# chacorp/latent-nerf-test

Hardware: AMD Instinct MI355X
Metric: latent-frames/sec (64x64x4, 128^3 grid), render forward+backward (higher is better)
Workload: dtype bf16

## Files before the change

include/lnerf_hip.h:

```cpp
#ifndef LNERF_HIP_H
#define LNERF_HIP_H

#include <stddef.h>
#include <stdint.h>

#ifdef __cplusplus
extern "C" {
#endif

#define LNERF_ABI_VERSION 7

#define LNERF_OK 0
#define LNERF_ERR_INVALID_ARG (-1)
#define LNERF_ERR_HIP (-2)
#define LNERF_ERR_UNSUPPORTED (-3)

#define LNERF_F32 0
#define LNERF_BF16 1

#define LNERF_MAX_LEVELS 32

typedef void *lnerf_stream_t;

int lnerf_abi_version(void);
// ... 115 lines not shown
                       float blob_scale, float blob_std, int64_t m_host, const int32_t *m_dev, const float *sigmas,
                       const float *dsigmas, const float *drgbs, float *dfeat, float *dw1, float *db1, float *dw2,
                       float *db2, float *dw3, float *db3, int accumulate, void *workspace, size_t workspace_bytes,
                       int precision, void *clear_ptr, size_t clear_bytes, lnerf_stream_t stream);

int lnerf_density_normals(const float *dxyz_enc, const float *xyzs, const float *sigmas, float blob_scale,
                          float blob_std, int64_t m_host, const int32_t *m_dev, float *grad_sigma, float *normals,
                          lnerf_stream_t stream);

int lnerf_opacity_entropy_grad(const float *weights_sum, int64_t N, float scale, float eps, float *grad,
                               lnerf_stream_t stream);

int lnerf_synthetic_guidance(const float *image, const float *targets, const int32_t *dirs, const float *weights,
                             int64_t n_views, int rays_per_view, int C, int n_buckets, int t_lo, int t_hi,
                             float noise_scale, uint32_t seed, const int32_t *step_dev, float *grad_image,
                             const float *weights_sum, float ent_scale, float ent_eps, float *grad_weights_sum,
                             lnerf_stream_t stream);

int lnerf_composite_rays_train_forward(const float *sigmas, const float *rgbs, const float *deltas,
                                       const int32_t *rays, int64_t N, int C, float T_thresh, const float *bg_color,
                                       float *weights_sum, float *depth, float *image, lnerf_stream_t stream);
int lnerf_composite_rays_train_backward(const float *grad_weights_sum, const float *grad_depth,
                                        const float *grad_image, const float *sigmas, const float *rgbs,
                                        const float *deltas, const int32_t *rays, const float *weights_sum,
                                        const float *depth, const float *image, const float *bg_color, int64_t N,
                                        int C, float T_thresh, float *grad_sigmas, float *grad_rgbs, float *grad_bg,
                                        lnerf_stream_t stream);

int lnerf_composite_rays_train_decode_forward(const float *sigmas, const float *latents, const float *deltas,
                                              const int32_t *rays, int64_t N, float T_thresh, const float *decoder,
                                              const float *bg_color, float *weights_sum, float *depth,
                                              float *latent_image, float *image, lnerf_stream_t stream);
int lnerf_composite_rays_train_decode_backward(const float *grad_weights_sum, const float *grad_depth,
                                               const float *grad_image, const float *sigmas, const float *latents,
                                               const float *deltas, const int32_t *rays, const float *weights_sum,
                                               const float *depth, const float *latent_image, const float *decoder,
                                               const float *bg_color, int64_t N, float T_thresh, float *grad_sigmas,
                                               float *grad_latents, float *grad_bg, float *grad_decoder,
                                               lnerf_stream_t stream);
int lnerf_decode_image(const float *latent_image, const float *weights_sum, const float *decoder, const float *bg_color,
                       int64_t N, float *image, lnerf_stream_t stream);

int lnerf_occ_cell_points(const uint32_t *indices, int64_t n, int cascade_level, int grid_size, float bound,
                          const float *noise, float *xyzs, lnerf_stream_t stream);
size_t lnerf_occ_sample_scratch_bytes(int64_t n_cells);
int lnerf_occ_sample(const float *grid_level, int64_t n_cells, int cascade_level, int grid_size, float bound,
                     int64_t n_rand, uint32_t seed, uint32_t step, int32_t *scratch, uint32_t *indices, float *xyzs,
                     lnerf_stream_t stream);
int lnerf_occ_update(float *grid_level, const uint32_t *indices, int64_t n, const float *new_sigmas, float decay,
                     uint32_t *scratch_cells, lnerf_stream_t stream);
int lnerf_occ_update_mean(float *grid_level, int64_t n_cells, const uint32_t *indices, int64_t n, const float *new_sigmas,
                          float decay, uint32_t *scratch_cells, float *mean_dev, float *scratch256,
                          lnerf_stream_t stream);
int lnerf_occ_mean(const float *grid, int64_t n, float *mean_dev, float *scratch256, lnerf_stream_t stream);

int lnerf_bg_forward(const float *dirs, int64_t N, const float *w1, const float *b1, const float *w2, const float *b2,
                     int C, float *out, lnerf_stream_t stream);
int lnerf_bg_backward(const float *dirs, int64_t N, const float *w1, const float *b1, const float *w2, const float *b2,
                      int C, const float *dout, float *dw1, float *db1, float *dw2, float *db2, lnerf_stream_t stream);

int lnerf_mesh_winding_number(const float *points, int64_t n, const float *triangles, int n_faces, float *out,
                              lnerf_stream_t stream);
int lnerf_mesh_distance(const float *points, int64_t n, const float *triangles, int n_faces, float *out,
                        lnerf_stream_t stream);

int lnerf_raster_prepare(const float *verts, int n_verts, const int32_t *faces, int n_faces, const float *cam_host,
                         float *face_z, float *face_xy, lnerf_stream_t stream);
int lnerf_rasterize(int H, int W, const float *face_z, const float *face_xy, int n_faces, int32_t *face_idx,
                    float *bary, lnerf_stream_t stream);
int lnerf_raster_prepare_batch(const float *verts, int n_verts, const int32_t *faces, int n_faces,
                               const float *cams_dev, int B, int H, int W, float *face_z, float *face_xy,
                               int16_t *face_box, lnerf_stream_t stream);
int lnerf_rasterize_batch(int B, int H, int W, const float *face_z, const float *face_xy, const int16_t *face_box,
                          int n_faces, int32_t *face_idx, float *bary, lnerf_stream_t stream);
int lnerf_interpolate_attributes(const int32_t *face_idx, const float *bary, const float *attr, int n_pixels, int D,
                                 float *feat, lnerf_stream_t stream);
int lnerf_interpolate_attributes_backward(const int32_t *face_idx, const float *bary, const float *dfeat,
                                          int n_pixels, int D, float *dattr, lnerf_stream_t stream);
int lnerf_texture_map_forward(const float *uv, const int32_t *face_idx, const float *texture, int n_pixels, int C,
                              int R, int mode, float *out, lnerf_stream_t stream);
int lnerf_texture_map_backward(const float *uv, const int32_t *face_idx, const float *dout, int n_pixels, int C, int R,
                               int mode, float *dtexture, lnerf_stream_t stream);

int lnerf_uv_footprint(const int32_t *face_idx, const float *face_xy, const float *face_z, const float *face_uv, int B,
                       int H, int W, int n_faces, float *rho, lnerf_stream_t stream);
int lnerf_mip_build(const float *texture, int C, int R, int L, float *pyramid, lnerf_stream_t stream);
int lnerf_mip_build_backward(float *dpyramid, int C, int R, int L, float *dtexture, lnerf_stream_t stream);
int lnerf_texture_mip_forward(const float *uv, const float *rho, const int32_t *face_idx, const float *texture,
                              const float *pyramid, int n_pixels, int C, int R, int L, float bias, float *out,
                              lnerf_stream_t stream);
int lnerf_texture_mip_backward(const float *uv, const float *rho, const int32_t *face_idx, const float *dout,
                               int n_pixels, int C, int R, int L, float bias, float *dtexture, float *dpyramid,
                               lnerf_stream_t stream);

int lnerf_adam_step(float *p, void *g, int grad_dtype, float *m, float *v, void *shadow_bf16, int64_t n, float lr,
                    float beta1, float beta2, float eps, int step, const int32_t *step_dev, float grad_scale,
                    int zero_grad, lnerf_stream_t stream);
int lnerf_adam_tick(int32_t *step_dev, lnerf_stream_t stream);
#define LNERF_ADAM_TICK 2
int lnerf_adam_step_multi(int count, float *const *p_host, float *const *g_host, float *const *m_host,
                          float *const *v_host, const int64_t *n_host, const float *lr_host, float beta1, float beta2,
                          float eps, int step, const int32_t *step_dev, float grad_scale, int zero_grad,
                          lnerf_stream_t stream);
int lnerf_adam_step_multi_shadow(int count, float *const *p_host, float *const *g_host, float *const *m_host,
                                 float *const *v_host, const int64_t *n_host, const float *lr_host, float beta1,
                                 float beta2, float eps, int step, const int32_t *step_dev, float grad_scale,
// ... 142 lines not shown
```

latent-nerf-test_amd/csrc/rays.hip:

```cpp
#include "common.h"

#include <math.h>
#include <string.h>

namespace lnerf {

__device__ __forceinline__ void pixel_ray(const float *__restrict__ c2w, int H, int W, float fx, float fy, float cx,
                                          float cy, int64_t g, float o[3], float d[3]) {
    const int b = (int)(g / ((int64_t)H * W));
    const int p = (int)(g - (int64_t)b * H * W);
    const int j = p / W, i = p - j * W;
    const float *m = c2w + (int64_t)b * 16;
    const float xs = ((float)i + 0.5f - cx) / fx;
    const float ys = ((float)j + 0.5f - cy) / fy;
    const float inv = 1.0f / sqrtf(xs * xs + ys * ys + 1.0f);
    const float d0 = xs * inv, d1 = ys * inv, d2 = inv;
#pragma unroll
    for (int r = 0; r < 3; ++r) {
        d[r] = d0 * m[r * 4 + 0] + d1 * m[r * 4 + 1] + d2 * m[r * 4 + 2];
        o[r] = m[r * 4 + 3];
    }
}
__global__ void __launch_bounds__(256) k_get_rays(const float *__restrict__ c2w, int B, int H, int W, float fx,
                                                  float fy, float cx, float cy, float *__restrict__ rays_o,
// ... 646 lines not shown
__global__ void __launch_bounds__(256) k_occ_update_apply(float *__restrict__ grid, unsigned int *__restrict__ scratch,
                                                          const uint32_t *__restrict__ indices, int64_t n, float decay) {
    for (int64_t i = (int64_t)blockIdx.x * blockDim.x + threadIdx.x; i < n; i += (int64_t)gridDim.x * blockDim.x) {
        const uint32_t idx = indices ? indices[i] : (uint32_t)i;
        const unsigned int m = atomicExch(&scratch[idx], 0u);
        if (!(m & 0x80000000u)) continue;
        const float old = grid[idx];
        if (old >= 0.f) grid[idx] = fmaxf(old * decay, __uint_as_float(m & 0x7FFFFFFFu));
    }
}

constexpr int OCC_MEAN_BLOCKS = 256;
__global__ void __launch_bounds__(256) k_occ_mean_partial(const float *__restrict__ grid, int64_t n,
                                                          float *__restrict__ partial) {
    __shared__ float s_w[4];
    float s = 0.f;
    for (int64_t i = (int64_t)blockIdx.x * blockDim.x + threadIdx.x; i < n; i += (int64_t)gridDim.x * blockDim.x)
        s += fmaxf(grid[i], 0.f);
    s = wave_sum(s);
    if (lane_id() == 0) s_w[threadIdx.x >> 6] = s;
    __syncthreads();
    if (threadIdx.x == 0) partial[blockIdx.x] = ((s_w[0] + s_w[1]) + s_w[2]) + s_w[3];
}
__global__ void __launch_bounds__(256) k_occ_apply_mean(float *__restrict__ grid, unsigned int *__restrict__ scratch,
                                                        int64_t n, float decay, float *__restrict__ partial) {
    __shared__ float s_w[4];
    float s = 0.f;
    for (int64_t i = (int64_t)blockIdx.x * blockDim.x + threadIdx.x; i < n; i += (int64_t)gridDim.x * blockDim.x) {
        float g = grid[i];
        const unsigned int m = scratch[i];
        if (m & 0x80000000u) {
            scratch[i] = 0u;
            if (g >= 0.f) {
                g = fmaxf(g * decay, __uint_as_float(m & 0x7FFFFFFFu));
                grid[i] = g;
            }
        }
        s += fmaxf(g, 0.f);
    }
    s = wave_sum(s);
    if (lane_id() == 0) s_w[threadIdx.x >> 6] = s;
    __syncthreads();
    if (threadIdx.x == 0) partial[blockIdx.x] = ((s_w[0] + s_w[1]) + s_w[2]) + s_w[3];
}
__global__ void __launch_bounds__(64) k_occ_mean_final(const float *__restrict__ partial, int blocks, float n,
                                                       float *__restrict__ mean) {
    if (threadIdx.x == 0) {
        float s = 0.f;
        for (int b = 0; b < blocks; ++b) s += partial[b];
        *mean = s / n;
    }
}

static MarchParams make_params(float bound, int cascade, int G, int max_steps, float dt_gamma) {
    MarchParams P;
    P.bound = bound;
    P.cascade = cascade;
    P.G = G;
    P.max_steps = max_steps;
    P.dt_gamma = dt_gamma;
    P.dt_min = (float)(2.0 * 1.7320508075688772 / (double)max_steps);
    P.dt_max = (float)(2.0 * 1.7320508075688772 * (double)(1 << (cascade - 1)) / (double)G);
    P.dt_uniform = fminf(fmaxf(0.0f, P.dt_min), P.dt_max);
    return P;
}

static int grid_for(int64_t n, int block = 256, int cap = 4096) {
    int64_t g = div_up(n, block);
    if (g < 1) g = 1;
    if (g > cap) g = cap;
    return (int)g;
}

}

using namespace lnerf;

extern "C" {

int lnerf_get_rays(const float *c2w, int B, int H, int W, float fx, float fy, float cx, float cy, float *rays_o,
                   float *rays_d, lnerf_stream_t stream) {
    LNERF_REQUIRE(c2w && rays_o && rays_d, "get_rays: null pointer");
    LNERF_REQUIRE(B > 0 && H > 0 && W > 0, "get_rays: B,H,W must be positive (got %d,%d,%d)", B, H, W);
    LNERF_REQUIRE(fx != 0.f && fy != 0.f, "get_rays: zero focal length");
    const int64_t total = (int64_t)B * H * W;
    hipLaunchKernelGGL(k_get_rays, dim3(grid_for(total)), dim3(256), 0, as_stream(stream), c2w, B, H, W, fx, fy, cx, cy,
                       rays_o, rays_d);
    LNERF_CHECK_LAUNCH("get_rays");
    return LNERF_OK;
}

int lnerf_near_far_from_aabb(const float *rays_o, const float *rays_d, int64_t N, float xmin, float ymin, float zmin,
                             float xmax, float ymax, float zmax, float min_near, float *nears, float *fars,
                             lnerf_stream_t stream) {
    LNERF_REQUIRE(N >= 0, "near_far_from_aabb: negative N");
    if (N == 0) return LNERF_OK;
    LNERF_REQUIRE(rays_o && rays_d && nears && fars, "near_far_from_aabb: null pointer");
    LNERF_REQUIRE(xmin <= xmax && ymin <= ymax && zmin <= zmax, "near_far_from_aabb: inverted aabb");
    const RayBox box{xmin, ymin, zmin, xmax, ymax, zmax, min_near};
    hipLaunchKernelGGL(k_near_far, dim3(grid_for(N)), dim3(256), 0, as_stream(stream), rays_o, rays_d, N, box, nears, fars);
    LNERF_CHECK_LAUNCH("near_far_from_aabb");
    return LNERF_OK;
}

int lnerf_morton3d(const int32_t *coords, int64_t n, uint32_t *indices, lnerf_stream_t stream) {
    LNERF_REQUIRE(n >= 0, "morton3d: negative n");
// ... 209 lines not shown
    if (n_rand == 0) return LNERF_OK;
    LNERF_REQUIRE(grid_level && scratch && indices && xyzs, "occ_sample: null pointer");
    const int n_blocks = (int)div_up(n_cells, (int64_t)OCC_BLOCK_CELLS);
    int32_t *counts = scratch, *total = scratch + n_blocks, *list = scratch + n_blocks + 1;
    hipStream_t s = as_stream(stream);
    hipLaunchKernelGGL(k_occ_count, dim3((unsigned)n_blocks), dim3(256), 0, s, grid_level, n_cells, counts);
    LNERF_CHECK_LAUNCH("occ_sample(count)");
    hipLaunchKernelGGL(k_occ_fill, dim3((unsigned)n_blocks), dim3(256), 0, s, grid_level, n_cells, counts, n_blocks, list, total);
    LNERF_CHECK_LAUNCH("occ_sample(fill)");
    const float mip_bound = fminf((float)(1 << cascade_level), bound);
    hipLaunchKernelGGL(k_occ_draw, dim3(grid_for(2 * n_rand)), dim3(256), 0, s, list, total, n_cells, n_rand, seed, step,
                       mip_bound, grid_size, indices, xyzs);
    LNERF_CHECK_LAUNCH("occ_sample(draw)");
    return LNERF_OK;
}

size_t lnerf_occ_sample_scratch_bytes(int64_t n_cells) {
    if (n_cells <= 0) return 0;
    return (size_t)(div_up(n_cells, (int64_t)OCC_BLOCK_CELLS) + 1 + n_cells) * sizeof(int32_t);
}

int lnerf_occ_update(float *grid_level, const uint32_t *indices, int64_t n, const float *new_sigmas, float decay,
                     uint32_t *scratch_cells, lnerf_stream_t stream) {
    LNERF_REQUIRE(n >= 0, "occ_update: negative n");
    if (n == 0) return LNERF_OK;
    LNERF_REQUIRE(grid_level && new_sigmas && scratch_cells, "occ_update: null pointer");
    hipStream_t s = as_stream(stream);
    hipLaunchKernelGGL(k_occ_update_max, dim3(grid_for(n)), dim3(256), 0, s, scratch_cells, indices, n, new_sigmas);
    LNERF_CHECK_LAUNCH("occ_update(max)");
    hipLaunchKernelGGL(k_occ_update_apply, dim3(grid_for(n)), dim3(256), 0, s, grid_level, scratch_cells, indices, n, decay);
    LNERF_CHECK_LAUNCH("occ_update(apply)");
    return LNERF_OK;
}

int lnerf_occ_update_mean(float *grid_level, int64_t n_cells, const uint32_t *indices, int64_t n, const float *new_sigmas,
                          float decay, uint32_t *scratch_cells, float *mean_dev, float *scratch256,
                          lnerf_stream_t stream) {
    LNERF_REQUIRE(n >= 0 && n_cells > 0, "occ_update_mean: bad sizes");
    LNERF_REQUIRE(grid_level && scratch_cells && mean_dev && scratch256 && (n == 0 || new_sigmas),
                  "occ_update_mean: null pointer");
    hipStream_t s = as_stream(stream);
    if (n > 0) {
        hipLaunchKernelGGL(k_occ_update_max, dim3(grid_for(n)), dim3(256), 0, s, scratch_cells, indices, n, new_sigmas);
        LNERF_CHECK_LAUNCH("occ_update_mean(max)");
    }
    hipLaunchKernelGGL(k_occ_apply_mean, dim3(OCC_MEAN_BLOCKS), dim3(256), 0, s, grid_level, scratch_cells, n_cells, decay,
                       scratch256);
    LNERF_CHECK_LAUNCH("occ_update_mean(apply)");
    hipLaunchKernelGGL(k_occ_mean_final, dim3(1), dim3(64), 0, s, scratch256, OCC_MEAN_BLOCKS, (float)n_cells, mean_dev);
    LNERF_CHECK_LAUNCH("occ_update_mean(final)");
    return LNERF_OK;
}

int lnerf_occ_mean(const float *grid, int64_t n, float *mean_dev, float *scratch256, lnerf_stream_t stream) {
    LNERF_REQUIRE(n > 0 && grid && mean_dev && scratch256, "occ_mean: bad arguments");
    hipLaunchKernelGGL(k_occ_mean_partial, dim3(OCC_MEAN_BLOCKS), dim3(256), 0, as_stream(stream), grid, n, scratch256);
    LNERF_CHECK_LAUNCH("occ_mean(partial)");
    hipLaunchKernelGGL(k_occ_mean_final, dim3(1), dim3(64), 0, as_stream(stream), scratch256, OCC_MEAN_BLOCKS, (float)n,
                       mean_dev);
    LNERF_CHECK_LAUNCH("occ_mean(final)");
    return LNERF_OK;
}

}
```

latent-nerf-test_amd/src/latent_nerf/configs/render_config.py:

```python
from typing import Optional
from dataclasses import dataclass
from typing import Tuple

from ..models.nerf_utils import NeRFType


@dataclass
class RenderConfig:
    cuda_ray: bool = True
    max_steps: int = 1024
    num_steps: int = 128
    upsample_steps: int = 0
    update_extra_interval: int = 16
    occ_device_sampling: bool = True
    max_ray_batch: int = 4096
    density_thresh: float = 10.0
    train_w: int = 64
    train_h: int = 64
    eval_w: int = 128
    eval_h: int = 128
    jitter_pose: bool = False
    bound: float = 1.0
    dt_gamma: float = 0.0
    min_near: float = 0.1
    radius_range: Tuple[float, float] = (1.0, 1.5)
    fovy_range: Tuple[float, float] = (40.0, 70.0)
    train_pose: Optional[Tuple[float, float, float, float]] = None
    dir_text: bool = True
    angle_overhead: float = 30.0
    angle_front: float = 60.0
    backbone: str = "grid"
    nerf_type: NeRFType = NeRFType.latent
    bg_radius: float = 0.0
    grid_size: int = 128
    mlp_precision: str = "auto"
    table_dtype: str = "auto"
    gridtype: str = "auto"
    gather_variant: int = 0
    scatter_variant: int = -1
    noise_seed: Optional[int] = 0x5EED
    max_samples: int = 0

    def layout(self) -> str:
        if self.gridtype not in ("auto", "hash", "tiled", "blocked"):
            raise ValueError("render.gridtype must be 'auto', 'hash', 'tiled' or 'blocked' (got %r)" % (self.gridtype,))
        return "hash" if self.gridtype == "auto" else self.gridtype

    def precision(self, name: str) -> str:
        v = getattr(self, name)
        if v not in ("auto", "f32", "bf16"):
            raise ValueError("render.%s must be 'auto', 'f32' or 'bf16' (got %r)" % (name, v))
        return "f32" if v == "auto" else v
```

latent-nerf-test_amd/src/latent_nerf/models/renderer.py:

```python
import math
import os

import torch
import torch.nn as nn

from ..raymarching import backend as _b
from ..raymarching import raymarching as rm
from ..raymarching.raymarching import _p, _stream


def _sample_pdf(bins, weights, n_samples, stratified):
    w = weights + 1e-5
    cdf = torch.cumsum(w / w.sum(-1, keepdim=True), -1)
    cdf = torch.cat([torch.zeros_like(cdf[:, :1]), cdf], -1)
    if stratified:
        u = torch.linspace(0.5 / n_samples, 1.0 - 0.5 / n_samples, n_samples, device=bins.device)
        u = u[None].expand(bins.shape[0], n_samples).contiguous()
    else:
        u = torch.rand(bins.shape[0], n_samples, device=bins.device)
    hi = torch.searchsorted(cdf, u, right=True).clamp(max=cdf.shape[-1] - 1)
    lo = (hi - 1).clamp(min=0)
    c0, c1 = torch.gather(cdf, 1, lo), torch.gather(cdf, 1, hi)
    b0, b1 = torch.gather(bins, 1, lo), torch.gather(bins, 1, hi)
    span = c1 - c0
# ... 15 lines not shown
        self.r = renderer

    def __enter__(self):
        r = self.r
        if r._shadow_state is None or r._shadow_state[0].device != r.density_grid.device:
            r._shadow_state = [getattr(r, n).clone() for n in self.NAMES]
        self.real = [r._buffers[n] for n in self.NAMES]
        for n, t in zip(self.NAMES, r._shadow_state):
            r._buffers[n] = t
        return r

    def __exit__(self, *exc):
        for n, t in zip(self.NAMES, self.real):
            self.r._buffers[n] = t
        return False


class NeRFRenderer(nn.Module):
    def __init__(self, cfg, latent_mode: bool = True):
        super().__init__()
        self.cfg = cfg
        self.latent_mode = latent_mode
        self.tuned = False
        self.bound = float(cfg.bound)
        self.cascade = 1 + math.ceil(math.log2(cfg.bound)) if cfg.bound > 1 else 1
        self.grid_size = int(cfg.grid_size)
        self.density_scale = 1.0
        self.min_near = cfg.min_near
        self.density_thresh = cfg.density_thresh
        self.bg_radius = cfg.bg_radius
        self.cuda_ray = cfg.cuda_ray
        aabb = torch.tensor([-self.bound] * 3 + [self.bound] * 3, dtype=torch.float32)
        self.register_buffer("aabb_train", aabb)
        self.register_buffer("aabb_infer", aabb.clone())
        G3 = self.grid_size ** 3
        self.register_buffer("density_grid", torch.zeros(self.cascade, G3))
        self.register_buffer("density_bitfield", torch.zeros(self.cascade * G3 // 8, dtype=torch.uint8))
        self.register_buffer("mean_density_dev", torch.zeros(1))
        self.mean_density = 0.0
        self.iter_density = 0
        self.local_step = 0
        self._march = None
        self._march_slots = [None, None]
        self._ray_slots = [None, None]
        self._march_key = None
        self._budget = None
        self.mean_count = 0
        self._noise_counter = None
        self._occ_scratch = None
        self._occ_cells = None
        self._occ_gen = None
        self._occ_seed = 0x0CC0
        self._occ_sample_ws = None
        self._bg_const = {}
        self._shadow_state = None

    def forward(self, x, d=None):
        raise NotImplementedError()

    def density(self, x):
        raise NotImplementedError()

    def field(self, xyzs, m_host, m_dev=None, level_stride=None):
        raise NotImplementedError()

    def background(self, d):
        raise NotImplementedError()

    def normal(self, x):
        raise NotImplementedError()

    def decode_points(self, latents):
        raise NotImplementedError()

    def density_normals(self, xyzs):
        raise NotImplementedError()

    SHADED = ("lambertian", "textureless")

    def _check_shading(self, shading, light_d=None, sampler="run_cuda", orient=False, normal_image=False):
        if normal_image and (shading not in self.SHADED or not self.training or sampler != "run_cuda" or self.tuned):
            raise ValueError("normal_image=True needs shading='lambertian' / 'textureless' in training mode on the "
                             "occupancy-marched renderer, not latent_tune (got shading=%r, %s mode, %s%s)"
                             % (shading, "training" if self.training else "evaluation", sampler,
                                ", latent_tune" if self.tuned else ""))
        if orient and (shading not in self.SHADED or not self.training or sampler != "run_cuda"):
            raise ValueError("orient=True needs shading='lambertian' / 'textureless' in training mode on the "
                             "occupancy-marched renderer (got shading=%r, %s mode, %s)"
                             % (shading, "training" if self.training else "evaluation", sampler))
        if shading in self.SHADED:
            if light_d is None:
                raise ValueError("shading must be 'albedo' or 'normal' unless light_d is given: shading=%r needs "
                                 "light_d=[3] / [B,3] (direction toward the light)" % (shading,))
            if sampler != "run_cuda":
                raise ValueError("shading=%r is built for the occupancy-marched renderer (cuda_ray = true); the uniform "
                                 "sampler renders 'albedo' and 'normal'" % (shading,))
            if self.tuned:
                raise ValueError("shading=%r is not available with render.nerf_type = latent_tune (the decoded colours "
                                 "are composited per ray)" % (shading,))
            return False, True
        if shading not in ("albedo", "normal"):
            raise ValueError("shading must be 'albedo', 'normal', or 'lambertian' / 'textureless' with light_d "
                             "(got %r)" % (shading,))
        if shading == "normal" and self.training:
            raise ValueError("shading='normal' is an evaluation render: call .eval() first (normals are not "
                             "differentiable here)")
# ... 425 lines not shown
        extra = {}
        if atlas == "charts":
            vt, ft, info = rm.chart_atlas(verts, faces, R)
            extra = {"face_chart": info["face_chart"], "chart_rect": info["chart_rect"], "atlas_scale": info["scale"]}
        else:
            need = atlas_min_resolution(F)
            if F > 0 and R < need:
                warnings.warn("export_mesh: texture_resolution %d gives the per-triangle atlas of %d faces %.1f texels per "
                              "chart cell (fewer than %d): use texture_resolution >= %d, or target_faces <= %d"
                              % (R, F, R / atlas_cells(F), MIN_TEXELS_PER_CELL, need, 2 * (R // MIN_TEXELS_PER_CELL) ** 2),
                              stacklevel=3)
            vt, ft = per_triangle_atlas(F, verts.device)
        baked = self.bake_texture(verts, faces, vt, ft, resolution=R, gutter=gutter, S=S)
        os.makedirs(path, exist_ok=True)
        out = os.path.join(path, "mesh.obj")
        write_textured_obj(out, verts.cpu().numpy(), faces.cpu().numpy(), vt.cpu().numpy(), ft.cpu().numpy(),
                           normals.cpu().numpy(), material="mesh.mtl", texture="albedo.png")
        albedo = (baked["rgb"].permute(1, 2, 0).cpu().numpy() * 255).round().astype(np.uint8)
        Image.fromarray(albedo).save(os.path.join(path, "albedo.png"))
        if (self.latent_mode or self.tuned) and baked["texture"].shape[0] == 4:
            torch.save(baked["texture"].cpu(), os.path.join(path, "latent_texture.pt"))
        if normal_map:
            nmap = self.bake_texture(verts, faces, vt, ft, resolution=R, gutter=gutter, S=S,
                                     fn=lambda pts: (self.normal(pts) + 1.0) / 2.0)["texture"]
            img = (nmap.clamp(0, 1).permute(1, 2, 0).cpu().numpy() * 255).round().astype(np.uint8)
            Image.fromarray(img).save(os.path.join(path, "normal_object.png"))
            baked = dict(baked, normal_map=nmap)
        return dict(baked, vt=vt, ft=ft, **extra)

    def shadow_extra_state(self):
        return _ShadowExtraState(self)

    def occupancy_generator(self, seed=None):
        dev = self.density_grid.device
        if seed is not None or self._occ_gen is None or self._occ_gen.device != dev:
            self._occ_gen = torch.Generator(device=dev)
            self._occ_gen.manual_seed(0x0CC0 + (0 if seed is None else int(seed)))
            if seed is not None:
                self._occ_seed = 0x0CC0 + int(seed)
        return self._occ_gen

    @torch.no_grad()
    def update_extra_state(self, decay=0.95, S=128):
        if not self.cuda_ray:
            return
        if self.training:
            self.update_sample_budget()
        dev = self.density_grid.device
        gen = self.occupancy_generator()
        G, G3 = self.grid_size, self.grid_size ** 3
        chunk = 1 << 20
        if self._occ_cells is None or self._occ_cells.device != dev:
            self._occ_cells = torch.zeros(G3, device=dev, dtype=torch.int32)
        fused_mean = False
        for cas in range(self.cascade):
            if self.iter_density >= 16 and getattr(self.cfg, "occ_device_sampling", True):
                n_rand = G3 // 4
                if self._occ_sample_ws is None or self._occ_sample_ws[0].device != dev:
                    nb = _b.get_lib().lnerf_occ_sample_scratch_bytes(G3)
                    self._occ_sample_ws = (torch.empty(nb, device=dev, dtype=torch.uint8),
                                           torch.empty(2 * n_rand, device=dev, dtype=torch.int32),
                                           torch.empty(2 * n_rand, 3, device=dev))
                scratch, idx, xyzs = self._occ_sample_ws
                level = self.density_grid[cas]
                _b.call("lnerf_occ_sample", _p(level), G3, cas, G, self.bound, n_rand, self._occ_seed & 0xFFFFFFFF,
                        (self.iter_density * 8 + cas) & 0xFFFFFFFF, _p(scratch), _p(idx), _p(xyzs), _stream())
                sigmas, _ = self.field(xyzs, 2 * n_rand)
                sigmas = sigmas.contiguous() if self.density_scale == 1.0 else (sigmas * self.density_scale).contiguous()
                if self.cascade == 1:
                    if self._occ_scratch is None or self._occ_scratch.device != dev:
                        self._occ_scratch = torch.zeros(256, device=dev)
                    _b.call("lnerf_occ_update_mean", _p(level), G3, _p(idx), 2 * n_rand, _p(sigmas), float(decay),
                            _p(self._occ_cells), _p(self.mean_density_dev), _p(self._occ_scratch), _stream())
                    fused_mean = True
                    continue
                _b.call("lnerf_occ_update", _p(level), _p(idx), 2 * n_rand, _p(sigmas), float(decay), _p(self._occ_cells),
                        _stream())
                continue
            if self.iter_density < 16:
                indices = None
                n = G3
            else:
                n_rand = G3 // 4
                rand_idx = torch.randint(0, G3, (n_rand,), device=dev, dtype=torch.int32, generator=gen)
                occ = torch.nonzero(self.density_grid[cas] > 0).squeeze(-1)
                if occ.numel() > 0:
                    pick = torch.randint(0, occ.numel(), (n_rand,), device=dev, generator=gen)
                    occ_idx = occ[pick].to(torch.int32)
                    indices = torch.cat([rand_idx, occ_idx])
                else:
                    indices = rand_idx
                n = indices.numel()
            level = self.density_grid[cas]
            for s in range(0, n, chunk):
                e = min(s + chunk, n)
                idx = None if indices is None else indices[s:e].contiguous()
                if idx is None:
                    idx = torch.arange(s, e, device=dev, dtype=torch.int32)
                noise = torch.rand(e - s, 3, device=dev, generator=gen)
                xyzs = torch.empty(e - s, 3, device=dev)
                _b.call("lnerf_occ_cell_points", _p(idx), e - s, cas, G, self.bound, _p(noise), _p(xyzs), _stream())
                sigmas, _ = self.field(xyzs, e - s)
                sigmas = (sigmas * self.density_scale).contiguous()
                _b.call("lnerf_occ_update", _p(level), _p(idx), e - s, _p(sigmas), float(decay), _p(self._occ_cells),
                        _stream())
        if not fused_mean:
            if self._occ_scratch is None or self._occ_scratch.device != dev:
                self._occ_scratch = torch.zeros(256, device=dev)
            _b.call("lnerf_occ_mean", _p(self.density_grid), self.density_grid.numel(), _p(self.mean_density_dev),
                    _p(self._occ_scratch), _stream())
        self.iter_density += 1
        rm.packbits(self.density_grid, self.density_thresh, self.density_bitfield, self.mean_density_dev)

    def render(self, rays_o, rays_d, staged=False, max_ray_batch=4096, **kwargs):
        _run = self.run_cuda if self.cuda_ray else self.run
        if not self.cuda_ray:
            kwargs.setdefault("num_steps", self.cfg.num_steps)
            kwargs.setdefault("upsample_steps", self.cfg.upsample_steps)
        if kwargs.get("prepared") is not None or (kwargs.get("camera") is not None and self.cuda_ray and self.training):
            kwargs.pop("force_all_rays", None)
            return self.run_cuda(None, None, **kwargs)
        camera = kwargs.pop("camera", None)
        if camera is not None and rays_o is None:
            poses, intr, him, wim = camera
            if torch.is_tensor(intr):
                intr = [float(v) for v in intr.reshape(-1)[:4].tolist()]
            rays_o, rays_d = rm.get_rays(poses, intr, int(him), int(wim))
        B, N = rays_o.shape[:2]
        if staged and not self.cuda_ray:
            dev = rays_o.device
            depth = torch.empty(B, N, device=dev)
            image = torch.empty(B, N, 3 if kwargs.get("shading", "albedo") == "normal" else self.img_dims, device=dev)
            wsum = torch.empty(B, N, device=dev)
            for b in range(B):
                for head in range(0, N, max_ray_batch):
                    tail = min(head + max_ray_batch, N)
                    r = _run(rays_o[b:b + 1, head:tail], rays_d[b:b + 1, head:tail], **kwargs)
                    depth[b:b + 1, head:tail] = r["depth"]
                    image[b:b + 1, head:tail] = r["image"]
                    wsum[b:b + 1, head:tail] = r["weights_sum"]
            return {"depth": depth, "image": image, "weights_sum": wsum}
        return _run(rays_o, rays_d, **kwargs)
```

latent-nerf-test_amd/src/latent_nerf/raymarching/backend.py:

```python
import ctypes
import os
import re

_HERE = os.path.dirname(os.path.abspath(__file__))
PKG_ROOT = os.path.abspath(os.path.join(_HERE, "..", "..", ".."))
REPO_ROOT = os.path.abspath(os.path.join(PKG_ROOT, ".."))
LIB_PATH = os.environ.get("LNERF_HIP_LIB", os.path.join(PKG_ROOT, "lib", "liblnerf_hip.so"))
HEADER_PATH = os.path.join(REPO_ROOT, "include", "lnerf_hip.h")

LNERF_OK = 0
F32, BF16 = 0, 1
MLP_FRAGMENTS_READY = 0x100
SCATTER_ZERO_HEAD_BYTES = 64 * 1024
MLP_FRAGMENT_BYTES = 36 * 1024
SCATTER_DEFER_FINISH = 0x200
MLP_DEFER_REDUCE = 0x200
TAIL_TICK, TAIL_CLEAR_SCATTER = 1, 2
GRID_BLOCKED = 0x400
GRID_TILED = 0x800
SCATTER_CLEARED = 0x100
MC_CLOSE_BOUNDARY, MC_COUNT_ONLY, MC_REUSE_COUNT = 1, 2, 4
UV_ITEMS, UV_COVER, UV_EMIT = 1, 2, 4
UV_MAX_RES = 8192
DECIMATE_DEFAULT_ROUNDS = 128
# ... 29 lines not shown
    "lnerf_build_info": [],
    "lnerf_set_tuning": [_c.c_char_p, _I],
    "lnerf_get_rays": [_P, _I, _I, _I, _F, _F, _F, _F, _P, _P, _P],
    "lnerf_near_far_from_aabb": [_P, _P, _L, _F, _F, _F, _F, _F, _F, _F, _P, _P, _P],
    "lnerf_morton3d": [_P, _L, _P, _P],
    "lnerf_morton3d_invert": [_P, _L, _P, _P],
    "lnerf_packbits": [_P, _L, _F, _P, _P, _P],
    "lnerf_march_rays_train": [_P, _P, _P, _P, _L, _P, _F, _I, _I, _I, _F, _P, _U, _P, _L, _P, _P, _P, _P, _P, _P],
    "lnerf_march_rays_train_aabb": [_P, _P, _F, _F, _F, _F, _F, _F, _F, _L, _P, _F, _I, _I, _I, _F, _P, _U, _P, _L, _P, _P,
                                    _P, _P, _P, _P],
    "lnerf_march_rays_train_pose": [_P, _I, _I, _I, _F, _F, _F, _F, _P, _P, _F, _F, _F, _F, _F, _F, _F, _P, _F, _I, _I, _I,
                                    _F, _P, _U, _P, _L, _P, _P, _P, _P, _P, _P],
    "lnerf_march_rays_train_camera": [_P, _P, _I, _I, _I, _P, _P, _F, _F, _F, _F, _F, _F, _F, _P, _F, _I, _I, _I, _F, _P, _U,
                                      _P, _L, _P, _P, _P, _P, _P, _P],
    "lnerf_march_rays": [_L, _I, _P, _P, _P, _P, _P, _P, _F, _I, _I, _I, _F, _P, _P, _P, _P],
    "lnerf_composite_rays": [_L, _I, _P, _P, _P, _P, _P, _I, _F, _P, _P, _P, _P, _P],
    "lnerf_compact_rays": [_P, _L, _P, _P, _P],
    "lnerf_grid_encode_forward": [_P, _F, _P, _I, _I, _I, _P, _P, _P, _L, _P, _L, _P, _I, _I, _P],
    "lnerf_grid_encode_backward_workspace_bytes": [_I, _P, _L],
    "lnerf_grid_encode_backward": [_P, _F, _P, _I, _I, _I, _P, _P, _P, _L, _P, _L, _P, _I, _P, _Z, _P],
    "lnerf_grid_encode_backward_bf16": [_P, _F, _P, _I, _I, _I, _P, _P, _P, _L, _P, _L, _P, _I, _P, _Z, _P, _P],
    "lnerf_grid_scatter_bin": [_P, _F, _P, _I, _I, _I, _P, _P, _P, _L, _P, _L, _P, _I, _P, _Z, _P],
    "lnerf_grid_scatter_reduce_bf16": [_F, _I, _I, _P, _P, _P, _L, _L, _I, _I, _P, _I, _P, _Z, _P, _P],
    "lnerf_grid_encode_backward_adam": [_P, _F, _P, _I, _I, _I, _P, _P, _P, _L, _P, _L, _P, _I, _P, _Z, _P, _P, _P, _P, _F,
                                        _F, _F, _F, _I, _P, _F, _P],
    "lnerf_grid_encode_backward_input": [_P, _F, _P, _I, _I, _I, _P, _P, _P, _L, _P, _L, _P, _P, _I, _P],
    "lnerf_grid_tv_plan": [_I, _P, _L, _P],
    "lnerf_grid_tv_lines": [_I, _P, _P, _U, _U, _P, _P, _P],
    "lnerf_grid_tv_grad": [_P, _I, _I, _P, _P, _I, _P, _P, _U, _U, _P, _P, _P, _P],
    "lnerf_density_normals": [_P, _P, _P, _F, _F, _L, _P, _P, _P, _P],
    "lnerf_mlp_forward": [_P, _I, _L, _P, _P, _P, _P, _P, _P, _P, _I, _F, _F, _L, _P, _P, _P, _I, _P, _Z, _P],
    "lnerf_mlp_backward_workspace_bytes": [_I],
    "lnerf_grid_scatter_clear_bytes": [_I, _P, _L],
    "lnerf_moment_map_bytes": [_I, _P],
    "lnerf_moment_map_build": [_P, _P, _I, _I, _P, _P, _Z, _P],
    "lnerf_moment_map_bind": [_P, _P, _Z],
    "lnerf_occ_sample_scratch_bytes": [_L],
    "lnerf_march_counter_len": [_L],
    "lnerf_occ_sample": [_P, _L, _I, _I, _F, _L, _U, _U, _P, _P, _P, _P],
    "lnerf_mlp_backward": [_P, _I, _L, _P, _P, _P, _P, _P, _P, _P, _I, _F, _F, _L, _P, _P, _P, _P, _P, _P, _P, _P,
                           _P, _P, _P, _I, _P, _Z, _I, _P, _Z, _P],
    "lnerf_composite_rays_train_forward": [_P, _P, _P, _P, _L, _I, _F, _P, _P, _P, _P, _P],
    "lnerf_composite_rays_train_backward": [_P, _P, _P, _P, _P, _P, _P, _P, _P, _P, _P, _L, _I, _F, _P, _P, _P, _P],
    "lnerf_composite_rays_train_decode_forward": [_P, _P, _P, _P, _L, _F, _P, _P, _P, _P, _P, _P, _P],
    "lnerf_composite_rays_train_decode_backward": [_P, _P, _P, _P, _P, _P, _P, _P, _P, _P, _P, _P, _L, _F, _P, _P, _P, _P,
                                                   _P],
    "lnerf_decode_image": [_P, _P, _P, _P, _L, _P, _P],
    "lnerf_opacity_entropy_grad": [_P, _L, _F, _F, _P, _P],
    "lnerf_synthetic_guidance": [_P, _P, _P, _P, _L, _I, _I, _I, _I, _I, _F, _U, _P, _P, _P, _F, _F, _P, _P],
    "lnerf_occ_cell_points": [_P, _L, _I, _I, _F, _P, _P, _P],
    "lnerf_occ_update": [_P, _P, _L, _P, _F, _P, _P],
    "lnerf_occ_mean": [_P, _L, _P, _P, _P],
    "lnerf_occ_update_mean": [_P, _L, _P, _L, _P, _F, _P, _P, _P, _P],
    "lnerf_bg_forward": [_P, _L, _P, _P, _P, _P, _I, _P, _P],
    "lnerf_bg_backward": [_P, _L, _P, _P, _P, _P, _I, _P, _P, _P, _P, _P, _P],
    "lnerf_mesh_winding_number": [_P, _L, _P, _I, _P, _P],
    "lnerf_mesh_distance": [_P, _L, _P, _I, _P, _P],
    "lnerf_raster_prepare": [_P, _I, _P, _I, _P, _P, _P, _P],
    "lnerf_rasterize": [_I, _I, _P, _P, _I, _P, _P, _P],
    "lnerf_raster_prepare_batch": [_P, _I, _P, _I, _P, _I, _I, _I, _P, _P, _P, _P],
    "lnerf_rasterize_batch": [_I, _I, _I, _P, _P, _P, _I, _P, _P, _P],
    "lnerf_interpolate_attributes": [_P, _P, _P, _I, _I, _P, _P],
    "lnerf_interpolate_attributes_backward": [_P, _P, _P, _I, _I, _P, _P],
    "lnerf_texture_map_forward": [_P, _P, _P, _I, _I, _I, _I, _P, _P],
    "lnerf_texture_map_backward": [_P, _P, _P, _I, _I, _I, _I, _P, _P],
    "lnerf_uv_footprint": [_P, _P, _P, _P, _I, _I, _I, _I, _P, _P],
    "lnerf_mip_build": [_P, _I, _I, _I, _P, _P],
    "lnerf_mip_build_backward": [_P, _I, _I, _I, _P, _P],
    "lnerf_texture_mip_forward": [_P, _P, _P, _P, _P, _I, _I, _I, _I, _F, _P, _P],
    "lnerf_texture_mip_backward": [_P, _P, _P, _P, _I, _I, _I, _I, _F, _P, _P, _P],
    "lnerf_adam_step": [_P, _P, _I, _P, _P, _P, _L, _F, _F, _F, _F, _I, _P, _F, _I, _P],
    "lnerf_adam_tick": [_P, _P],
    "lnerf_adam_step_multi": [_I, _P, _P, _P, _P, _P, _P, _F, _F, _F, _I, _P, _F, _I, _P],
    "lnerf_adam_step_multi_shadow": [_I, _P, _P, _P, _P, _P, _P, _F, _F, _F, _I, _P, _F, _I, _P, _P, _P],
    "lnerf_mlp_fragment_maps": [_I, _P, _P, _P, _P],
    "lnerf_cast_f32_to_bf16": [_P, _P, _L, _P],
    "lnerf_mlp_backward_slabs": [_L, _I],
    "lnerf_grid_encode_backward_adam_tail": [_P, _F, _P, _I, _I, _I, _P, _P, _P, _L, _P, _L, _P, _I, _P, _Z, _P, _P, _P, _P,
                                             _F, _P, _Z, _I, _I, _P, _P, _P, _F, _P, _F, _F, _F, _I, _P, _F, _I, _P],
    "lnerf_marching_cubes_scratch_bytes": [_I, _I, _I, _I],
    "lnerf_marching_cubes": [_P, _I, _I, _I, _F, _F, _F, _F, _F, _F, _F, _I, _P, _Z, _P, _P, _L, _P, _L, _P, _P],
    "lnerf_uv_raster_scratch_bytes": [_I, _I],
    "lnerf_uv_raster": [_P, _I, _P, _P, _I, _P, _I, _I, _I, _L, _P, _Z, _P, _P, _P, _L, _P, _P],
    "lnerf_uv_dilate": [_P, _P, _I, _I, _I, _P, _P, _P],
    "lnerf_decimate_scratch_bytes": [_I, _I],
    "lnerf_decimate": [_P, _I, _P, _I, _I, _F, _I, _P, _Z, _P, _P, _P, _P, _P],
    "lnerf_atlas_buckets": [_P, _I, _P, _I, _P, _P, _P, _P],
    "lnerf_atlas_round": [_P, _P, _I, _P, _P, _P],
    "lnerf_atlas_compact_scratch_bytes": [_I],
    "lnerf_atlas_compact": [_P, _P, _I, _P, _Z, _P, _P, _P, _P],
    "lnerf_atlas_boxes_scratch_bytes": [_I],
    "lnerf_atlas_boxes": [_P, _I, _P, _P, _P, _I, _I, _P, _Z, _P, _P],
    "lnerf_atlas_uv": [_P, _I, _P, _P, _I, _P, _P, _P, _P, _I, _I, _F, _I, _P, _I, _P],
    "lnerf_atlas_fold_scratch_bytes": [_I, _I],
    "lnerf_atlas_fold": [_P, _I, _P, _I, _I, _I, _L, _P, _Z, _P, _P, _P, _P],
    "lnerf_mesh_components_begin": [_P, _I, _I, _P, _P, _P],
    "lnerf_mesh_components_round": [_P, _I, _I, _P, _P, _P],
    "lnerf_mesh_components_scratch_bytes": [_I, _I],
    "lnerf_mesh_components_finish": [_P, _I, _P, _I, _P, _P, _Z, _P, _P, _P, _P, _P, _P],
    "lnerf_mesh_filter_scratch_bytes": [_I, _I],
    "lnerf_mesh_filter": [_P, _I, _I, _P, _P, _Z, _P, _P, _P, _P],
    "lnerf_mesh_smooth_scratch_bytes": [_I, _I],
    "lnerf_mesh_smooth": [_P, _I, _P, _I, _I, _F, _F, _P, _Z, _P, _P, _P],
    "lnerf_fd_points": [_P, _F, _F, _L, _P, _P, _P, _P],
    "lnerf_shade_fd_forward": [_P, _P, _I, _P, _L, _I, _P, _I, _F, _P, _P, _P],
    "lnerf_shade_fd_backward": [_P, _P, _I, _P, _L, _I, _P, _I, _F, _P, _P, _P, _P, _P],
# ... 87 lines not shown
```

Before: 2794.

## Use stratified pull-based occupancy update and fuse mean into packbits

```diff
diff --git a/include/lnerf_hip.h b/include/lnerf_hip.h
--- a/include/lnerf_hip.h
+++ b/include/lnerf_hip.h
@@ -191,6 +191,11 @@
 int lnerf_occ_update_mean(float *grid_level, int64_t n_cells, const uint32_t *indices, int64_t n, const float *new_sigmas,
                           float decay, uint32_t *scratch_cells, float *mean_dev, float *scratch256,
                           lnerf_stream_t stream);
+int lnerf_occ_update_mean_stratified(float *grid_level, int64_t n_cells, const uint32_t *indices, int64_t n,
+                                     const float *new_sigmas, float decay, uint32_t *scratch_cells, float *mean_dev,
+                                     float *scratch256, int64_t n_rand, const int32_t *total_dev, lnerf_stream_t stream);
+int lnerf_packbits_partials(const float *grid, int64_t n_cells, float thresh, const float *partial256, float *mean_dev,
+                            uint8_t *bitfield, lnerf_stream_t stream);
 int lnerf_occ_mean(const float *grid, int64_t n, float *mean_dev, float *scratch256, lnerf_stream_t stream);
 
 int lnerf_bg_forward(const float *dirs, int64_t N, const float *w1, const float *b1, const float *w2, const float *b2,
diff --git a/latent-nerf-test_amd/csrc/rays.hip b/latent-nerf-test_amd/csrc/rays.hip
--- a/latent-nerf-test_amd/csrc/rays.hip
+++ b/latent-nerf-test_amd/csrc/rays.hip
@@ -722,6 +722,122 @@
     }
 }
 
+__global__ void __launch_bounds__(256) k_occ_run_max(unsigned int *__restrict__ scratch,
+                                                     const uint32_t *__restrict__ indices, int64_t n_rand,
+                                                     const float *__restrict__ sig, const int32_t *__restrict__ total_dev) {
+    if (*total_dev <= 0) return;
+    const int lane = lane_id();
+    const int64_t n_up = (n_rand + 255) / 256 * 256;
+    for (int64_t k = (int64_t)blockIdx.x * blockDim.x + threadIdx.x; k < n_up; k += (int64_t)gridDim.x * blockDim.x) {
+        const bool in = k < n_rand;
+        const uint32_t idx = in ? indices[n_rand + k] : 0xFFFFFFFFu;
+        const uint32_t next = (k + 1 < n_rand) ? indices[n_rand + k + 1] : 0xFFFFFFFFu;
+        const float s = in ? sig[n_rand + k] : -1.0f;
+        unsigned int v = (s >= 0.f) ? (__float_as_uint(s) | 0x80000000u) : 0u;
+#pragma unroll
+        for (int d = 1; d < 64; d <<= 1) {
+            const unsigned int ov = (unsigned int)__shfl_up((int)v, d, 64);
+            const uint32_t oi = (uint32_t)__shfl_up((int)idx, d, 64);
+            if (lane >= d && oi == idx) v = v > ov ? v : ov;
+        }
+        if (in && v != 0u && (lane == 63 || next != idx)) atomicMax(&scratch[idx], v);
+    }
+}
+__device__ __forceinline__ unsigned int occ_pull_word(const uint32_t *__restrict__ indices, const float *__restrict__ sig,
+                                                      int64_t j, uint32_t cell) {
+    const float c = sig[j];
+    return (indices[j] == cell && c >= 0.f) ? (__float_as_uint(c) | 0x80000000u) : 0u;
+}
+__device__ __forceinline__ float occ_apply_cell(float *__restrict__ grid, unsigned int *__restrict__ scratch, int64_t i,
+                                                float g, unsigned int held, unsigned int m, float decay) {
+    m = m > held ? m : held;
+    if (held & 0x80000000u) scratch[i] = 0u;
+    if ((m & 0x80000000u) && g >= 0.f) {
+        g = fmaxf(g * decay, __uint_as_float(m & 0x7FFFFFFFu));
+        grid[i] = g;
+    }
+    return fmaxf(g, 0.f);
+}
+constexpr int OCC_APPLY_TRIPS = 8;
+template <bool SECOND>
+__device__ __forceinline__ float occ_apply_slice(float *__restrict__ grid, unsigned int *__restrict__ scratch, int64_t n,
+                                                 float decay, const uint32_t *__restrict__ indices, int64_t n_rand,
+                                                 const float *__restrict__ sig) {
+    const int64_t stride = (int64_t)gridDim.x * blockDim.x;
+    float s = 0.f;
+    int64_t i = (int64_t)blockIdx.x * blockDim.x + threadIdx.x;
+    for (; i + (OCC_APPLY_TRIPS - 1) * stride < n; i += OCC_APPLY_TRIPS * stride) {
+        float g[OCC_APPLY_TRIPS];
+        unsigned int held[OCC_APPLY_TRIPS], m[OCC_APPLY_TRIPS];
+#pragma unroll
+        for (int u = 0; u < OCC_APPLY_TRIPS; ++u) {
+            const int64_t c = i + u * stride;
+            g[u] = grid[c];
+            held[u] = scratch[c];
+            m[u] = occ_pull_word(indices, sig, c >> 2, (uint32_t)c);
+            if (SECOND) {
+                const unsigned int v = occ_pull_word(indices, sig, n_rand + (c >> 2), (uint32_t)c);
+                m[u] = m[u] > v ? m[u] : v;
+            }
+        }
+#pragma unroll
+        for (int u = 0; u < OCC_APPLY_TRIPS; ++u) s += occ_apply_cell(grid, scratch, i + u * stride, g[u], held[u], m[u], decay);
+    }
+    for (; i < n; i += stride) {
+        unsigned int m = occ_pull_word(indices, sig, i >> 2, (uint32_t)i);
+        if (SECOND) {
+            const unsigned int v = occ_pull_word(indices, sig, n_rand + (i >> 2), (uint32_t)i);
+            m = m > v ? m : v;
+        }
+        s += occ_apply_cell(grid, scratch, i, grid[i], scratch[i], m, decay);
+    }
+    return s;
+}
+__global__ void __launch_bounds__(256) k_occ_apply_mean_pull(float *__restrict__ grid, unsigned int *__restrict__ scratch,
+                                                             int64_t n, float decay, float *__restrict__ partial,
+                                                             const uint32_t *__restrict__ indices, int64_t n_rand,
+                                                             const float *__restrict__ sig,
+                                                             const int32_t *__restrict__ total_dev) {
+    __shared__ float s_w[4];
+    float s = *total_dev <= 0 ? occ_apply_slice<true>(grid, scratch, n, decay, indices, n_rand, sig)
+                              : occ_apply_slice<false>(grid, scratch, n, decay, indices, n_rand, sig);
+    s = wave_sum(s);
+    if (lane_id() == 0) s_w[threadIdx.x >> 6] = s;
+    __syncthreads();
+    if (threadIdx.x == 0) partial[blockIdx.x] = ((s_w[0] + s_w[1]) + s_w[2]) + s_w[3];
+}
+__global__ void __launch_bounds__(256) k_packbits_partials(const float *__restrict__ grid, int64_t n_bytes, float thresh,
+                                                           const float *__restrict__ partial, float n,
+                                                           float *__restrict__ mean, uint8_t *__restrict__ bits) {
+    static_assert(OCC_MEAN_BLOCKS == 4 * 64, "one float4 per lane");
+    const float4 p = reinterpret_cast<const float4 *>(partial)[lane_id()];
+    float s = 0.f;
+#pragma unroll
+    for (int l = 0; l < 64; ++l) {
+        s += __int_as_float(__builtin_amdgcn_readlane(__float_as_int(p.x), l));
+        s += __int_as_float(__builtin_amdgcn_readlane(__float_as_int(p.y), l));
+        s += __int_as_float(__builtin_amdgcn_readlane(__float_as_int(p.z), l));
+        s += __int_as_float(__builtin_amdgcn_readlane(__float_as_int(p.w), l));
+    }
+    const float m = s / n;
+    if (blockIdx.x == 0 && threadIdx.x == 0) *mean = m;
+    const float th = fminf(thresh, m);
+    for (int64_t b = (int64_t)blockIdx.x * blockDim.x + threadIdx.x; b < n_bytes; b += (int64_t)gridDim.x * blockDim.x) {
+        const float4 lo = reinterpret_cast<const float4 *>(grid)[b * 2];
+        const float4 hi = reinterpret_cast<const float4 *>(grid)[b * 2 + 1];
+        uint32_t v = 0;
+        v |= (lo.x > th) ? 1u : 0u;
+        v |= (lo.y > th) ? 2u : 0u;
+        v |= (lo.z > th) ? 4u : 0u;
+        v |= (lo.w > th) ? 8u : 0u;
+        v |= (hi.x > th) ? 16u : 0u;
+        v |= (hi.y > th) ? 32u : 0u;
+        v |= (hi.z > th) ? 64u : 0u;
+        v |= (hi.w > th) ? 128u : 0u;
+        bits[b] = (uint8_t)v;
+    }
+}
+
 static MarchParams make_params(float bound, int cascade, int G, int max_steps, float dt_gamma) {
     MarchParams P;
     P.bound = bound;
@@ -1037,6 +1153,43 @@
     return LNERF_OK;
 }
 
+int lnerf_occ_update_mean_stratified(float *grid_level, int64_t n_cells, const uint32_t *indices, int64_t n,
+                                     const float *new_sigmas, float decay, uint32_t *scratch_cells, float *mean_dev,
+                                     float *scratch256, int64_t n_rand, const int32_t *total_dev, lnerf_stream_t stream) {
+    LNERF_REQUIRE(n_rand > 0 && n_cells <= ((int64_t)1 << 31), "occ_update_mean_stratified: bad sizes");
+    LNERF_REQUIRE(n == 2 * n_rand && n_cells == 4 * n_rand,
+                  "occ_update_mean_stratified: needs n == 2 * n_rand and n_cells == 4 * n_rand (got n %lld, n_cells %lld, "
+                  "n_rand %lld): other lists go through lnerf_occ_update_mean",
+                  (long long)n, (long long)n_cells, (long long)n_rand);
+    LNERF_REQUIRE(grid_level && indices && new_sigmas && scratch_cells && scratch256 && total_dev,
+                  "occ_update_mean_stratified: null pointer");
+    hipStream_t s = as_stream(stream);
+    hipLaunchKernelGGL(k_occ_run_max, dim3(grid_for(n_rand)), dim3(256), 0, s, scratch_cells, indices, n_rand, new_sigmas,
+                       total_dev);
+    LNERF_CHECK_LAUNCH("occ_update_mean_stratified(runs)");
+    hipLaunchKernelGGL(k_occ_apply_mean_pull, dim3(OCC_MEAN_BLOCKS), dim3(256), 0, s, grid_level, scratch_cells, n_cells,
+                       decay, scratch256, indices, n_rand, new_sigmas, total_dev);
+    LNERF_CHECK_LAUNCH("occ_update_mean_stratified(apply)");
+    if (mean_dev) {
+        hipLaunchKernelGGL(k_occ_mean_final, dim3(1), dim3(64), 0, s, scratch256, OCC_MEAN_BLOCKS, (float)n_cells, mean_dev);
+        LNERF_CHECK_LAUNCH("occ_update_mean_stratified(final)");
+    }
+    return LNERF_OK;
+}
+
+int lnerf_packbits_partials(const float *grid, int64_t n_cells, float thresh, const float *partial256, float *mean_dev,
+                            uint8_t *bitfield, lnerf_stream_t stream) {
+    LNERF_REQUIRE(n_cells > 0 && n_cells % 8 == 0, "packbits_partials: n_cells (%lld) must be a positive multiple of 8",
+                  (long long)n_cells);
+    LNERF_REQUIRE(grid && partial256 && mean_dev && bitfield, "packbits_partials: null pointer");
+    LNERF_REQUIRE((((uintptr_t)grid | (uintptr_t)partial256) & 15) == 0,
+                  "packbits_partials: grid and partial256 must be 16-byte aligned");
+    hipLaunchKernelGGL(k_packbits_partials, dim3(grid_for(n_cells / 8, 256, 512)), dim3(256), 0, as_stream(stream), grid,
+                       n_cells / 8, thresh, partial256, (float)n_cells, mean_dev, bitfield);
+    LNERF_CHECK_LAUNCH("packbits_partials");
+    return LNERF_OK;
+}
+
 int lnerf_occ_mean(const float *grid, int64_t n, float *mean_dev, float *scratch256, lnerf_stream_t stream) {
     LNERF_REQUIRE(n > 0 && grid && mean_dev && scratch256, "occ_mean: bad arguments");
     hipLaunchKernelGGL(k_occ_mean_partial, dim3(OCC_MEAN_BLOCKS), dim3(256), 0, as_stream(stream), grid, n, scratch256);
diff --git a/latent-nerf-test_amd/src/latent_nerf/configs/render_config.py b/latent-nerf-test_amd/src/latent_nerf/configs/render_config.py
--- a/latent-nerf-test_amd/src/latent_nerf/configs/render_config.py
+++ b/latent-nerf-test_amd/src/latent_nerf/configs/render_config.py
@@ -13,6 +13,7 @@
     upsample_steps: int = 0
     update_extra_interval: int = 16
     occ_device_sampling: bool = True
+    occ_stratified_update: bool = True
     max_ray_batch: int = 4096
     density_thresh: float = 10.0
     train_w: int = 64
diff --git a/latent-nerf-test_amd/src/latent_nerf/models/renderer.py b/latent-nerf-test_amd/src/latent_nerf/models/renderer.py
--- a/latent-nerf-test_amd/src/latent_nerf/models/renderer.py
+++ b/latent-nerf-test_amd/src/latent_nerf/models/renderer.py
@@ -91,6 +91,7 @@
         self._occ_gen = None
         self._occ_seed = 0x0CC0
         self._occ_sample_ws = None
+        self._occ_total = None
         self._bg_const = {}
         self._shadow_state = None
 
@@ -622,7 +623,7 @@
         chunk = 1 << 20
         if self._occ_cells is None or self._occ_cells.device != dev:
             self._occ_cells = torch.zeros(G3, device=dev, dtype=torch.int32)
-        fused_mean = False
+        fused_mean = mean_in_packbits = False
         for cas in range(self.cascade):
             if self.iter_density >= 16 and getattr(self.cfg, "occ_device_sampling", True):
                 n_rand = G3 // 4
@@ -631,15 +632,21 @@
                     self._occ_sample_ws = (torch.empty(nb, device=dev, dtype=torch.uint8),
                                            torch.empty(2 * n_rand, device=dev, dtype=torch.int32),
                                            torch.empty(2 * n_rand, 3, device=dev))
+                    self._occ_total = self._occ_sample_ws[0][nb - 4 * (G3 + 1):]
                 scratch, idx, xyzs = self._occ_sample_ws
                 level = self.density_grid[cas]
                 _b.call("lnerf_occ_sample", _p(level), G3, cas, G, self.bound, n_rand, self._occ_seed & 0xFFFFFFFF,
                         (self.iter_density * 8 + cas) & 0xFFFFFFFF, _p(scratch), _p(idx), _p(xyzs), _stream())
                 sigmas, _ = self.field(xyzs, 2 * n_rand)
                 sigmas = sigmas.contiguous() if self.density_scale == 1.0 else (sigmas * self.density_scale).contiguous()
+                if self._occ_scratch is None or self._occ_scratch.device != dev:
+                    self._occ_scratch = torch.zeros(256, device=dev)
+                if getattr(self.cfg, "occ_stratified_update", True):
+                    _b.call("lnerf_occ_update_mean_stratified", _p(level), G3, _p(idx), 2 * n_rand, _p(sigmas), float(decay),
+                            _p(self._occ_cells), None, _p(self._occ_scratch), n_rand, _p(self._occ_total), _stream())
+                    mean_in_packbits = self.cascade == 1
+                    continue
                 if self.cascade == 1:
-                    if self._occ_scratch is None or self._occ_scratch.device != dev:
-                        self._occ_scratch = torch.zeros(256, device=dev)
                     _b.call("lnerf_occ_update_mean", _p(level), G3, _p(idx), 2 * n_rand, _p(sigmas), float(decay),
                             _p(self._occ_cells), _p(self.mean_density_dev), _p(self._occ_scratch), _stream())
                     fused_mean = True
@@ -674,12 +681,16 @@
                 sigmas = (sigmas * self.density_scale).contiguous()
                 _b.call("lnerf_occ_update", _p(level), _p(idx), e - s, _p(sigmas), float(decay), _p(self._occ_cells),
                         _stream())
+        self.iter_density += 1
+        if mean_in_packbits:
+            _b.call("lnerf_packbits_partials", _p(self.density_grid), G3, float(self.density_thresh), _p(self._occ_scratch),
+                    _p(self.mean_density_dev), _p(self.density_bitfield), _stream())
+            return
         if not fused_mean:
             if self._occ_scratch is None or self._occ_scratch.device != dev:
                 self._occ_scratch = torch.zeros(256, device=dev)
             _b.call("lnerf_occ_mean", _p(self.density_grid), self.density_grid.numel(), _p(self.mean_density_dev),
                     _p(self._occ_scratch), _stream())
-        self.iter_density += 1
         rm.packbits(self.density_grid, self.density_thresh, self.density_bitfield, self.mean_density_dev)
 
     def render(self, rays_o, rays_d, staged=False, max_ray_batch=4096, **kwargs):
diff --git a/latent-nerf-test_amd/src/latent_nerf/raymarching/backend.py b/latent-nerf-test_amd/src/latent_nerf/raymarching/backend.py
--- a/latent-nerf-test_amd/src/latent_nerf/raymarching/backend.py
+++ b/latent-nerf-test_amd/src/latent_nerf/raymarching/backend.py
@@ -105,6 +105,8 @@
     "lnerf_occ_update": [_P, _P, _L, _P, _F, _P, _P],
     "lnerf_occ_mean": [_P, _L, _P, _P, _P],
     "lnerf_occ_update_mean": [_P, _L, _P, _L, _P, _F, _P, _P, _P, _P],
+    "lnerf_occ_update_mean_stratified": [_P, _L, _P, _L, _P, _F, _P, _P, _P, _L, _P, _P],
+    "lnerf_packbits_partials": [_P, _L, _F, _P, _P, _P, _P],
     "lnerf_bg_forward": [_P, _L, _P, _P, _P, _P, _I, _P, _P],
     "lnerf_bg_backward": [_P, _L, _P, _P, _P, _P, _I, _P, _P, _P, _P, _P, _P],
     "lnerf_mesh_winding_number": [_P, _L, _P, _I, _P, _P],
```

New measurement: 2804, median of 6. No clear change (+0.3%).
